# nnethercott/hannoy

Measured on AMD Instinct MI355X. Metric: vectors indexed/sec (build) + recall@10, 1M x 768 Cosine M=16 efC=100, higher is better.
Workload: dtype f32

## Files before the change

hannoy_amd/csrc/hny_host.cpp:

```cpp
#include "../../include/hannoy_amd.h"
#include "hny_internal.h"
#include "hny_rust_sort.h"

#include <malloc.h>
#include <algorithm>
#include <array>
#include <atomic>
#include <mutex>
#include <chrono>
#include <cmath>
#include <cstdarg>
#include <cstdio>
#include <cstdlib>
#include <cstring>
#include <functional>
#include <iterator>
#include <memory>
#include <numeric>
#include <string>
#include <thread>
#include <type_traits>
#include <utility>
#include <vector>

// ... 289 lines not shown
  std::vector<int8_t> ins_level;
  std::vector<uint16_t> old_mask;
  std::vector<uint8_t> deleted;
  std::vector<u64> old_recs;
  bool incremental = false;
  bool load_only = false;
  bool gaps_done = false;
  bool from_update = false;
  uint64_t n_done0 = 0;
  uint32_t up_layers = 1;
  std::vector<uint32_t> entry_points;
  std::vector<uint64_t> rec_first;
  std::vector<uint32_t> rec_item_t;
  std::vector<uint8_t> rec_layer_t;
  std::vector<int32_t> upper_idx;
  uint32_t max_level = 0, n_upper = 0;
  LaunchShape shape{64, 1};
  double frac = 0.0;
  uint32_t bmax = 0;
  int device = 0;
  hipStream_t stream = nullptr;
  std::vector<hipEvent_t> sync_evs;
  size_t sync_used = 0;
  size_t pos = 0;
  uint64_t n_done = 0, n_batches = 0;
  hny_batch cur{};
  bool in_batch = false, finalized = false;
  GraphDev g{};
  DevBuf<unsigned char> d_rows, d_level;
  DevBuf<float> d_norms, d_l0_dist, d_up_dist;
  DevBuf<int> d_upper_idx;
  DevBuf<u32> d_l0_ids, d_l0_cnt, d_up_ids, d_up_cnt, d_order, d_eps, d_bits, d_vlog, d_cand_n,
      d_seg_start, d_nseg, d_deferred, d_deferred_b, d_fin_cnt0, d_fin_cntu, d_d0_ids, d_du_ids;
  DevBuf<unsigned char> d_has_vec, d_deleted;
  DevBuf<u64> d_old_recs, d_lkey_a, d_lkey_b, d_perm_a, d_perm_b;
  DevBuf<u32> d_gap_bitmap, d_gap_bm;
  DevBuf<u64> d_gap_keys, d_gap_sorted;
  int gap_grid = 0;
  DevBuf<u32> d_eps0;
  DevBuf<u32> d_pool_retry, d_pool_retry2, d_pool_ctr;
  DevBuf<u64> d_heap_c, d_heap_r;
  uint32_t heap_grid = 0, heap_c_cap = 0, heap_r_cap = 0, pool_ctr_used = 0;
  uint32_t heap_grid1 = 0, heap_c_cap1 = 0;
  u64 *heap_c_ptr = nullptr;
  struct ExportBufs : ExportSlots {
    std::thread th;
    void join() {
      if (th.joinable()) th.join();
    }
    void drop() {
      join();
      drop_all();
    }
    ~ExportBufs() { drop(); }
  } xbuf;
  bool will_export = true;
  std::vector<uint32_t> item_slot;
  uint64_t n_items = 0;
  std::unique_ptr<IngestPipe> qpipe;
  uint64_t nrec_bound = 0, nbr_bound = 0;
  bool locality = true;
  u32 *h_l0 = nullptr, *h_up = nullptr, *h_cnt0 = nullptr, *h_cntu = nullptr;
  DevBuf<u64> d_stats, d_stats_scratch, d_sel, d_cand, d_res_global;
  DevBuf<u64> d_ops;
  struct { u64 *p = nullptr; size_t n = 0; } d_keys_a, d_keys_b, d_vals_a, d_vals_b;
  DevBuf<unsigned char> d_sort_tmp;
// ... 122 lines not shown
  for (uint32_t v : set)
    if (c <= v) {
      s.lpr = (int)l;
      s.nch = (int)v;
      return HNY_OK;
    }
  return fail(HNY_ERR_UNSUPPORTED, "dim %u needs more than 16 chunks per lane (max f32 dim 4096)", dim);
}

int mclass_of(int metric) {
  switch (metric) {
    case HNY_COSINE: return MC_DOT;
    case HNY_EUCLIDEAN: return MC_L2;
    case HNY_MANHATTAN: return MC_L1;
    default: return MC_BIN;
  }
}

uint32_t cap_of(const hny_builder *b, uint32_t layer_or_level) {
  return layer_or_level == 0 ? b->o.M0 : b->o.M;
}

int env_int(const char *name, int dflt) {
  const char *v = getenv(name);
  return v && *v ? atoi(v) : dflt;
}

Knobs knobs_from_env() {
  Knobs k{};
  k.no_fast = env_int("HNY_NO_FAST", 0) != 0;
  k.no_rb = env_int("HNY_NO_RB", 0) != 0;
  k.rb_one = env_int("HNY_RB_ONE", 1) != 0;
  k.prune_n8 = env_int("HNY_PRUNE_N8", 1) != 0;
  k.walk_slots = env_int("HNY_WALK_SLOTS", HNY_KNOB_UNSET);
  k.xcd_tile = env_int("HNY_XCD_TILE", HNY_KNOB_UNSET);
  k.prune_xcd_tile = env_int("HNY_PRUNE_XCD_TILE", HNY_KNOB_UNSET);
  k.walk_resident = env_int("HNY_WALK_RESIDENT", HNY_KNOB_UNSET);
  k.visited_log = env_int("HNY_VISITED_LOG", HNY_KNOB_UNSET);
  k.vis_slots = env_int("HNY_VIS_SLOTS", HNY_KNOB_UNSET);
  k.stage_bytes = env_int("HNY_STAGE_BYTES", HNY_KNOB_UNSET);
  k.no_locality = env_int("HNY_NO_LOCALITY", 0) != 0;
  k.heap_small_cap = env_int("HNY_HEAP_SMALL_CAP", HNY_KNOB_UNSET);
  k.vis_buckets = env_int("HNY_VIS_BUCKETS", HNY_KNOB_UNSET);
  return k;
}

int upload_rows(const void *vectors, size_t stride, size_t vbytes, uint64_t n, uint32_t row_stride,
                unsigned char *dst, hipStream_t st, const uint32_t *slots = nullptr, uint64_t n_slots = 0) {
  if (!slots) n_slots = n;
  if (!slots && stride == row_stride && vbytes == row_stride) {
    HIP_TRY(hipMemcpyAsync(dst, vectors, (size_t)n * row_stride, hipMemcpyHostToDevice, st));
    HIP_TRY(hipStreamSynchronize(st));
    return HNY_OK;
  }
  const size_t chunk_rows = std::max<size_t>(1, (64u << 20) / row_stride);
  std::vector<unsigned char> stage(chunk_rows * row_stride);
  uint64_t r = 0;
  for (uint64_t s0 = 0; s0 < n_slots; s0 += chunk_rows) {
    size_t cnt = (size_t)std::min<uint64_t>(chunk_rows, n_slots - s0);
    std::fill(stage.begin(), stage.begin() + cnt * row_stride, 0);
    for (; r < n && (slots ? slots[r] : r) < s0 + cnt; r++)
      memcpy(&stage[((slots ? slots[r] : r) - s0) * row_stride], (const unsigned char *)vectors + r * stride, vbytes);
    HIP_TRY(hipMemcpyAsync(dst + s0 * row_stride, stage.data(), cnt * row_stride,
                           hipMemcpyHostToDevice, st));
    HIP_TRY(hipStreamSynchronize(st));
  }
// ... 112 lines not shown
    a.out_hdrs = j.out_hdrs ? p.d_hdrs[k] : nullptr;
    HIP_TRY(hnyk_ingest(a, st));
    HIP_TRY(hipEventRecord(p.consumed[k], st));
    p.used[k] = true;
    if (j.out_codes)
      HIP_TRY(hipMemcpyAsync((unsigned char *)j.out_codes + r0 * vb, p.d_codes[k], (size_t)cnt * vb, hipMemcpyDeviceToHost, st));
    if (j.out_hdrs)
      HIP_TRY(hipMemcpyAsync((unsigned char *)j.out_hdrs + r0 * hb, p.d_hdrs[k], (size_t)cnt * hb, hipMemcpyDeviceToHost, st));
  }
  return HNY_OK;
}

int check_f32_rows(uint32_t dim, uint64_t n, const void *vectors, size_t stride) {
  if (dim == 0) return fail(HNY_ERR_INVALID_DIM, "dim must be > 0");
  if (n && !vectors) return fail(HNY_ERR_INVALID_ARG, "null f32 vectors");
  if (n && stride < (size_t)dim * 4)
    return fail(HNY_ERR_INVALID_DIM, "stride %zu < %zu bytes of f32 for dim %u", stride, (size_t)dim * 4, dim);
  if (n && stride % 4) return fail(HNY_ERR_INVALID_ARG, "f32 stride %zu is not a multiple of 4", stride);
  return HNY_OK;
}

int reset_graph(hny_builder *b) {
  hipStream_t st = b->stream;
  HIP_TRY(hnyk_fill_u32(b->d_l0_ids.p, HNY_SENT, b->d_l0_ids.n, st));
  HIP_TRY(hipMemsetAsync(b->d_l0_cnt.p, 0, b->d_l0_cnt.n * 4, st));
  HIP_TRY(hipMemsetAsync(b->d_l0_dist.p, 0, b->d_l0_dist.n * 4, st));
  if (b->d_up_ids.n) {
    HIP_TRY(hnyk_fill_u32(b->d_up_ids.p, HNY_SENT, b->d_up_ids.n, st));
    HIP_TRY(hipMemsetAsync(b->d_up_cnt.p, 0, b->d_up_cnt.n * 4, st));
    HIP_TRY(hipMemsetAsync(b->d_up_dist.p, 0, b->d_up_dist.n * 4, st));
  }
  HIP_TRY(hipMemsetAsync(b->d_stats.p, 0, ST_COUNT * 8, st));
  HIP_TRY(hipMemsetAsync(b->d_bits.p, 0, b->d_bits.n * 4, st));
  b->pos = 0;
  b->n_done = b->n_done0;
  b->n_batches = 0;
  b->in_batch = false;
  b->finalized = false;
  b->gaps_done = false;
  b->ev_used = 0;
  b->n_walk_dispatch = 0;
  b->sync_used = 0;
  b->t_build0 = now_s();
  return HNY_OK;
}

int use_device(int device) {
  int ndev = 0;
  if (hipGetDeviceCount(&ndev) != hipSuccess || ndev == 0)
    return fail(HNY_ERR_NO_DEVICE, "no HIP device (this library has no CPU path)");
  if (device >= 0) HIP_TRY(hipSetDevice(device));
  return HNY_OK;
}

size_t group_end(const hny_builder *b, size_t pos) {
  size_t e = pos;
  while (e < b->order.size() && b->order_level[e] == b->order_level[pos]) e++;
  return e;
}

inline uint32_t rec_mask_of(const hny_builder *b, uint32_t s) {
  if (b->deleted[s]) return 0u;
  uint32_t m = b->old_mask[s];
  if (b->ins_level[s] >= 0) m |= (2u << b->ins_level[s]) - 1u;
  return m;
}
// ... 751 lines not shown
    const uint64_t area = b->heap_c_ptr == b->d_ops.p ? b->d_ops.n : b->d_heap_c.n;
    const uint64_t small_cap = (uint64_t)std::max(16, knob_or(b->knobs.heap_small_cap, 1 << 18));
    if ((uint64_t)b->heap_c_cap > small_cap) {
      b->heap_c_cap1 = (uint32_t)small_cap;
      b->heap_grid1 = (uint32_t)std::max<uint64_t>(1, std::min<uint64_t>(std::min<uint64_t>(slots, 512), area / small_cap));
      HIP_TRY(b->d_pool_retry2.alloc(cand_rows));
    }
    HIP_TRY(b->d_heap_r.alloc((size_t)std::max(b->heap_grid, b->heap_grid1) * b->heap_r_cap));
    HIP_TRY(b->d_pool_retry.alloc(cand_rows));
    HIP_TRY(b->d_pool_ctr.alloc(4 * 64));
  }
  HIP_TRY(b->d_deferred.alloc(b->max_ops));
  HIP_TRY(b->d_deferred_b.alloc(b->max_ops));
  {
    u32 tbits = 1;
    while ((1ull << tbits) < (u64)b->n + 1ull) tbits++;
    const u32 ranges[3][2] = {{0, 64}, {HNY_SEQ_BITS, 64}, {HNY_SEQ_BITS, (u32)HNY_SEQ_BITS + tbits}};
    b->sort_tmp_bytes = 0;
    for (size_t sz = b->max_ops; sz >= 1; sz = sz > 1 ? sz / 2 : 0) {
      for (auto &r : ranges) {
        size_t need = 0;
        HIP_TRY(hnyk_sort_pairs(nullptr, need, b->d_keys_a.p, b->d_keys_b.p, b->d_vals_a.p, b->d_vals_b.p,
                                (u32)sz, r[0], r[1], st));
        b->sort_tmp_bytes = std::max(b->sort_tmp_bytes, need);
      }
      size_t need = 0;
      HIP_TRY(hnyk_sort_pairs48(nullptr, need, b->d_keys_a.p, b->d_keys_b.p, b->d_vals_a.p, b->d_vals_b.p,
                                (u32)sz, st));
      b->sort_tmp_bytes = std::max(b->sort_tmp_bytes, need);
      need = 0;
      HIP_TRY(hnyk_sort_u32(nullptr, need, b->d_deferred.p, b->d_deferred_b.p, (u32)sz, st));
      b->sort_tmp_bytes = std::max(b->sort_tmp_bytes, need);
      if (sz == 1) break;
    }
  }
  HIP_TRY(b->d_sort_tmp.alloc(b->sort_tmp_bytes + 16));
  if (b->incremental && n) {
    HIP_TRY(b->d_d0_ids.alloc((size_t)n * o.M0));
    HIP_TRY(b->d_du_ids.alloc(std::max<size_t>(nup * o.M, 1)));
    HIP_TRY(b->d_has_vec.alloc(n));
    HIP_TRY(b->d_deleted.alloc(n));
    HIP_TRY(b->d_old_recs.alloc(std::max<size_t>(b->old_recs.size(), 1)));
  }

  GraphDev &g = b->g;
  const size_t vb = vec_bytes(o.metric, o.dim);
  g.n = n;
  g.metric = o.metric;
  g.mclass = mclass_of(o.metric);
  g.row_stride = row_stride;
  g.bin_bits = (u32)(vb * 8);
  g.bin_inv = (g.bin_bits && (g.bin_bits & (g.bin_bits - 1)) == 0) ? 1.0f / (float)g.bin_bits : 0.0f;
  g.M = o.M;
  g.M0 = o.M0;
  g.max_level = b->max_level;
  g.up_layers = b->up_layers;
  g.n_upper = b->n_upper;
  g.alpha = o.alpha;
  g.incremental = b->incremental ? 1 : 0;
  g.dim = o.dim;
  g.x86_order = o.x86_order ? 1 : 0;
  g.rows = b->d_rows.p;
  g.norms = b->d_norms.p;
  g.level = b->d_level.p;
  g.upper_idx = b->d_upper_idx.p;
  g.l0_ids = b->d_l0_ids.p;
// ... 375 lines not shown
      prof_end(b);
      PruneArgs p = prune_args(l, lo, hi);
      p.perm = b->d_perm_b.p;
      prof_begin(b, EV_PRUNE);
      HIP_TRY(launch_prune(p, b->stream));
      prof_end(b);
    }
    return HNY_OK;
  }
  for (int32_t l = (int32_t)L; l >= 0; l--) {
    WalkArgs w = walk_args(l, lo, hi, queues + l);
    prof_begin(b, EV_WALK);
    b->n_walk_dispatch++;
    HIP_TRY(launch_walk(w, b->stream));
    prof_end(b);
    prof_begin(b, EV_PRUNE);
    HIP_TRY(launch_prune(prune_args(l, lo, hi), b->stream));
    prof_end(b);
  }
  return HNY_OK;
}

static int apply_front(hny_builder *b, const void *sel_dev, ApplyArgs &a) {
  const uint32_t L = b->cur.level, cs = cap_of(b, L);
  const u64 *sel = sel_dev ? (const u64 *)sel_dev : b->d_sel.p;
  const u32 n_ops = b->cur.count * (L + 1) * cs * 2;
  EmitArgs e{};
  e.q_slots = b->d_order.p + b->cur.first;
  e.count = b->cur.count;
  e.sel = sel;
  e.sel_stride = b->cur.sel_stride_u64;
  e.cap_sel = cs;
  e.batch_level = L;
  e.keys = b->d_keys_a.p;
  e.vals = b->d_vals_a.p;
  prof_begin(b, EV_SORT);
  HIP_TRY(hnyk_emit(b->g, e, b->stream));
  size_t tmp = b->sort_tmp_bytes;
  HIP_TRY(hnyk_sort_pairs(b->d_sort_tmp.p, tmp, b->d_keys_a.p, b->d_keys_b.p, b->d_vals_a.p,
                          b->d_vals_b.p, n_ops, 0, 64, b->stream));
  HIP_TRY(hipMemsetAsync(b->d_nseg.p, 0, 8, b->stream));
  HIP_TRY(hnyk_segments(b->d_keys_b.p, n_ops, b->d_seg_start.p, b->d_nseg.p, b->stream));
  prof_end(b);
  a = ApplyArgs{};
  a.keys = b->d_keys_b.p;
  a.vals = b->d_vals_b.p;
  a.n_ops = n_ops;
  a.seg_start = b->d_seg_start.p;
  a.n_seg = b->d_nseg.p;
  a.deferred = b->apply_form.kind == APPLY_WAVE ? nullptr : b->d_deferred.p;
  a.n_deferred = b->d_nseg.p + 1;
  prof_begin(b, EV_APPLY);
  if (a.deferred) {
    HIP_TRY(hnyk_apply_append(b->g, a, b->stream));
  } else {
    const int grid = (int)std::min<u32>(std::max<u32>(n_ops / 2, 1), b->apply_form.grid_cap);
    HIP_TRY(hnyk_apply(b->g, a, b->shape, b->apply_form, grid, b->stream));
  }
  prof_end(b);
  b->cur_n_ops = n_ops;
  return HNY_OK;
}

static void apply_back(hny_builder *b) {
  b->pos += b->cur.count;
  b->n_done += b->cur.count;
  b->n_batches++;
  b->in_batch = false;
  b->apply_open = false;
}

int hny_builder_apply(hny_builder *b, const void *sel_dev) {
  if (!b || !b->in_batch || b->apply_open) return fail(HNY_ERR_INVALID_ARG, "no current batch");
  HIP_TRY(hipSetDevice(b->device));
  ApplyArgs a;
// ... 2592 lines not shown
```

hannoy_amd/csrc/hny_internal.h:

```cpp
#pragma once
#include <hip/hip_runtime.h>
#include <stddef.h>
#include <stdint.h>

typedef unsigned long long u64;
typedef unsigned int u32;

#define HNY_SENT 0xFFFFFFFFu
#define HNY_MAX_CAP 64
#define HNY_BIG_CAP 1024
#define HNY_MAX_EPS 8192
#define HNY_POOL_CAP 128
#define HNY_MAX_EF 65535
#define HNY_OP_INVALID 0xFFFFFFFFFFFFFFFFull
#define HNY_SEQ_BITS 29
#define HNY_MAX_LEVEL 14

enum { MC_DOT = 0, MC_L2 = 1, MC_L1 = 2, MC_BIN = 3 };

enum {
  ST_EVALS_WALK = 0,
  ST_EVALS_PRUNE = 1,
  ST_EVALS_APPLY = 2,
  ST_LINKS = 3,
// ... 144 lines not shown
  u32 count;
  const u64 *sel;
  u32 sel_stride, cap_sel, batch_level;
  u64 *keys;
  u64 *vals;
};

struct ApplyArgs {
  const u64 *keys;
  const u64 *vals;
  u32 n_ops;
  const u32 *seg_start;
  const u32 *n_seg;
  u32 *deferred;
  u32 *n_deferred;
  u32 shard_rank, shard_world;
  u64 *exch;
  u32 exch_stride;
};

struct LaunchShape {
  int lpr;
  int nch;
};

#define HNY_KNOB_UNSET (-2147483647 - 1)
struct Knobs {
  int no_fast;
  int no_rb;
  int rb_one;
  int prune_n8;
  int walk_slots, xcd_tile, prune_xcd_tile, walk_resident, visited_log, vis_slots, stage_bytes, no_locality,
      heap_small_cap, vis_buckets;
};
static inline int knob_or(int v, int dflt) { return v == HNY_KNOB_UNSET ? dflt : v; }

#ifndef HNY_RB_MAX_NCH
#define HNY_RB_MAX_NCH 3
#endif
#ifndef HNY_WALK_WPE
#define HNY_WALK_WPE 4
#endif
#ifndef HNY_WALK_WPE_SMALL
#define HNY_WALK_WPE_SMALL 6
#endif
constexpr int hnyk_walk_waves_per_simd(int lpr, int nch, int sp, bool rm, int rc) {
  return nch == 1 && sp >= 4 && !rm && (rc == 1 || rc == 2) && lpr <= 32 ? HNY_WALK_WPE_SMALL : HNY_WALK_WPE;
}

static inline bool hnyk_fast_path(const GraphDev &g, const Knobs &k) {
  return !k.no_fast && !g.x86_order && !g.incremental && g.metric >= 0 && g.metric < 7 && g.M0 <= 64u;
}
struct WalkForm {
  int sp;
  bool big_eps;
  bool reader;
  int rc;
  int waves_per_simd;
};
static inline WalkForm hnyk_walk_form(const GraphDev &g, const WalkArgs &a, LaunchShape s, const Knobs &k) {
  WalkForm f{0, a.eps_cap > 64, false, 0, 0};
  if (hnyk_fast_path(g, k) && a.eps_cap <= 64 && !a.res_global) {
    f.sp = g.metric + 1;
    f.reader = a.reader_mode != 0;
    if (s.nch <= HNY_RB_MAX_NCH && a.rcap <= 128 && !k.no_rb)
      f.rc = s.nch == 1 && s.lpr <= 32 && !f.reader && a.rb_one && k.rb_one ? 1 : 2;
// ... 81 lines not shown
  const u32 *filter_of;
  const u32 *masks;
  u32 mask_stride;
  const u32 *k_of;
  u32 *tile_mask;
};
static inline u32 hnyk_exact_qt(u32 row_stride) {
  u32 qt = 32;
  while (qt > 4 && (size_t)qt * row_stride > 65536u) qt /= 2;
  return qt;
}
hipError_t hnyk_exact_scores(const GraphDev &g, const ExactArgs &a, LaunchShape s, hipStream_t st);
hipError_t hnyk_exact_topk(const GraphDev &g, const ExactArgs &a, hipStream_t st);
hipError_t hnyk_exact_tile_masks(const ExactArgs &a, hipStream_t st);
struct RangeArgs {
  const float *scores;
  u32 score_stride;
  u32 nq;
  u32 slab_base, slab_n;
  const u32 *mask;
  const float *radius;
  u64 *count;
  u64 *keys;
  const u32 *seg;
  u32 *cursor;
};
hipError_t hnyk_range_count(const RangeArgs &a, hipStream_t st);
hipError_t hnyk_range_emit(const RangeArgs &a, hipStream_t st);
hipError_t hnyk_range_sort(void *temp, size_t &temp_bytes, u64 *keys, u64 *other, u32 n, u32 n_seg, const u32 *seg,
                           u64 **sorted, hipStream_t st);
hipError_t hnyk_range_finish(const u64 *keys, u32 n, const u32 *item_ids, u32 *ids, u32 *dist_bits, hipStream_t st);
hipError_t hnyk_emit(const GraphDev &g, const EmitArgs &a, hipStream_t st);
hipError_t hnyk_segments(const u64 *keys, u32 n_ops, u32 *seg_start, u32 *n_seg, hipStream_t st);
hipError_t hnyk_apply(const GraphDev &g, const ApplyArgs &a, LaunchShape s, const ApplyForm &f, int grid, hipStream_t st);
hipError_t hnyk_apply_append(const GraphDev &g, const ApplyArgs &a, hipStream_t st);
hipError_t hnyk_apply_deferred(const GraphDev &g, const ApplyArgs &a, LaunchShape s, const ApplyForm &f, StageRows sl,
                               u32 work, hipStream_t st);
hipError_t hnyk_apply_merge(const GraphDev &g, const u64 *exch, u32 n_def, u32 world, u32 rank, u32 per,
                            u32 stride, hipStream_t st);
hipError_t hnyk_sort_u32(void *temp, size_t &temp_bytes, u32 *in, u32 *out, u32 n, hipStream_t st);
hipError_t hnyk_sort_pairs(void *temp, size_t &temp_bytes, u64 *keys_in, u64 *keys_out, u64 *vals_in,
                           u64 *vals_out, u32 n, u32 begin_bit, u32 end_bit, hipStream_t st);
hipError_t hnyk_sort_pairs48(void *temp, size_t &temp_bytes, u64 *keys_in, u64 *keys_out, u64 *vals_in,
                             u64 *vals_out, u32 n, hipStream_t st);
hipError_t hnyk_iota_u64(u64 *p, u32 base, u32 n, hipStream_t st);
hipError_t hnyk_take_topk(const u64 *cand, const u32 *cand_n, u32 rcap, u32 k, u32 n, u64 *out,
                          hipStream_t st);
hipError_t hnyk_lane_selftest(u32 *out64, hipStream_t st);
hipError_t hnyk_pair_distances(const GraphDev &g, const u32 *a, const u32 *b, u32 n, float *out,
                               LaunchShape s, hipStream_t st);
hipError_t hnyk_fill_u32(u32 *p, u32 v, size_t n, hipStream_t st);
hipError_t hnyk_fill_gaps_wg(const GraphDev &g, const u64 *recs, u32 n_recs, const unsigned char *deleted,
                             u32 *bitmaps, u32 words, u32 *bm, u32 maxb, u64 *keys, u64 *sorted, int SL, int grid,
                             LaunchShape s, hipStream_t st);
hipError_t hnyk_fill_gaps(const GraphDev &g, const u64 *recs, u32 n_recs, const unsigned char *deleted,
                          LaunchShape s, hipStream_t st);
hipError_t hnyk_finalize_lists(u32 *ids, u32 *cnt_out, u32 n_lists, u32 cap, hipStream_t st);
size_t hnyk_walk_lds_bytes(u32 rcap, u32 eps_cap);
#define HNY_DECL_SP(N)                                                                                         \
  hipError_t hnyk_walk_sp##N(const GraphDev &g, const WalkArgs &a, LaunchShape s, const WalkForm &f, int grid, \
                             hipStream_t st);                                                                  \
  hipError_t hnyk_prune_sp##N(const GraphDev &g, const PruneArgs &a, LaunchShape s, const PruneForm &f, int SL, \
                              int grid, hipStream_t st);                                                       \
  hipError_t hnyk_apply_sp##N(const GraphDev &g, const ApplyArgs &a, LaunchShape s, const ApplyForm &f, int SL, \
                              int grid, hipStream_t st);
HNY_DECL_SP(1) HNY_DECL_SP(2) HNY_DECL_SP(3) HNY_DECL_SP(4) HNY_DECL_SP(5) HNY_DECL_SP(6) HNY_DECL_SP(7)
// ... 59 lines not shown
```

hannoy_amd/csrc/hny_kernels.hip:

```cpp
#include "hny_internal.h"

#include <algorithm>
#include <cstdlib>
#include <cstring>
#ifndef HNY_PART
#define HNY_PART 0
#endif
#if HNY_PART == 0
#include <rocprim/device/device_radix_sort.hpp>
#endif

#ifdef HNY_WSYNC_BARRIER
#define WSYNC() __syncthreads()
#else
#define WSYNC()                                               \
  do {                                                        \
    __builtin_amdgcn_fence(__ATOMIC_RELEASE, "workgroup");    \
    __builtin_amdgcn_wave_barrier();                          \
    __builtin_amdgcn_fence(__ATOMIC_ACQUIRE, "workgroup");    \
  } while (0)
#endif

#ifndef HNY_RB_MERGE
#define HNY_RB_MERGE 1
#endif
#ifndef HNY_RB_MERGE_MIN
#define HNY_RB_MERGE_MIN 2
#endif

#define HNY_LANE ((int)(threadIdx.x & 63u))

namespace {

__device__ __forceinline__ u32 fbits(float f) { return __float_as_uint(f); }
__device__ __forceinline__ u64 ballot(bool p) { return __builtin_amdgcn_ballot_w64(p); }

template <int SP>
__device__ __forceinline__ void specialize(GraphDev &g) {
  if constexpr (SP != 0) {
    g.metric = SP - 1;
    g.mclass = SP - 1 < 3 ? SP - 1 : (int)MC_BIN;
    g.x86_order = 0;
    g.incremental = 0;
  }
}
__device__ __forceinline__ u32 uni(u32 x) { return (u32)__builtin_amdgcn_readfirstlane((int)x); }
__device__ __forceinline__ u64 uni64(u64 x) { return ((u64)uni((u32)(x >> 32)) << 32) | (u64)uni((u32)x); }
__device__ __forceinline__ int uni(int x) { return __builtin_amdgcn_readfirstlane(x); }
__device__ __forceinline__ u64 uni(u64 x) {
  return ((u64)uni((u32)(x >> 32)) << 32) | (u64)uni((u32)(x & 0xFFFFFFFFull));
}

template <int LPR, int NCH>
__device__ __forceinline__ void load_row(const unsigned char *p, int t, u32 n16, float4 (&r)[NCH]) {
// ... 3283 lines not shown
    for (int j = 0; j < 4; j++) k[j + 1] = i0 + (u32)j < n_ops ? keys[i0 + j] : HNY_OP_INVALID;
    u32 flags = 0u;
#pragma unroll
    for (int j = 0; j < 4; j++) {
      const bool start = k[j + 1] != HNY_OP_INVALID &&
                         ((i0 + (u32)j) == 0u || (k[j] >> HNY_SEQ_BITS) != (k[j + 1] >> HNY_SEQ_BITS));
      flags |= (start ? 1u : 0u) << j;
    }
    const u32 c = (u32)__popc(flags);
    u32 incl = c;
#pragma unroll
    for (int off = 1; off < 64; off <<= 1) {
      const u32 t = (u32)__shfl_up((int)incl, off, 64);
      if (ln >= off) incl += t;
    }
    if (ln == 63) wsum[w] = incl;
    __syncthreads();
    u32 wbase = 0u, total = 0u;
#pragma unroll
    for (int j = 0; j < 4; j++) {
      if (j < w) wbase += wsum[j];
      total += wsum[j];
    }
    if (tid == 0) base_s = total ? atomicAdd(n_seg, total) : 0u;
    __syncthreads();
    u32 pos = base_s + wbase + incl - c;
#pragma unroll
    for (int j = 0; j < 4; j++)
      if ((flags >> j) & 1u) seg_start[pos++] = i0 + (u32)j;
    __syncthreads();
  }
}

__global__ __launch_bounds__(256) void k_apply_append(GraphDev g, ApplyArgs a) {
  const u32 n_seg = *a.n_seg;
  for (u32 sg = blockIdx.x * blockDim.x + threadIdx.x; sg < n_seg; sg += gridDim.x * blockDim.x) {
    const u32 i0 = a.seg_start[sg];
    const u64 k0 = a.keys[i0] >> HNY_SEQ_BITS;
    const u32 target = (u32)(k0 & 0x7FFFFFFFull);
    const NodeList l = node_list(g, (u32)(k0 >> 31), target);
    const u32 cw = *l.cnt;
    if (cw >> 31) continue;
    u32 cnt = cw & 0xFFFFu;
    u32 nops = 0;
    for (u32 i = i0; i < a.n_ops; i++) {
      const u64 key = a.keys[i];
      if (key == HNY_OP_INVALID || (key >> HNY_SEQ_BITS) != k0) break;
      nops++;
      if (cnt + nops > l.cap) break;
    }
    if (cnt + nops > l.cap) {
      a.deferred[atomicAdd(a.n_deferred, 1u)] = i0;
      continue;
    }
    for (u32 i = i0; i < i0 + nops; i++) {
      const u64 val = a.vals[i];
      if ((u32)(val & 0xFFFFFFFFull) == target) continue;
      l.ids[cnt] = (u32)(val & 0xFFFFFFFFull);
      l.dist[cnt] = __uint_as_float((u32)(val >> 32));
      cnt++;
    }
    *l.cnt = cnt;
  }
}

template <int LPR, int NCH, int SP>
// ... 776 lines not shown
                               u32 work, hipStream_t st) {
  const int SL = f.kind == APPLY_APPEND_N8 ? sl.n8 : sl.wg, grid = (int)std::min<u32>(work, f.grid_cap);
  HNY_SP_SWITCH(f.sp, hnyk_apply_sp, g, a, s, f, SL, grid, st)
  return dispatch_shape<Hot<0>::Apply>(s, g, a, f, SL, grid, st);
}
hipError_t hnyk_pair_distances(const GraphDev &g, const u32 *a, const u32 *b, u32 n, float *out,
                               LaunchShape s, hipStream_t st) {
  return dispatch_shape<PairLauncher>(s, g, a, b, n, out, st);
}
hipError_t hnyk_fill_gaps(const GraphDev &g, const u64 *recs, u32 n_recs, const unsigned char *deleted,
                          LaunchShape s, hipStream_t st) {
  if (!n_recs) return hipSuccess;
  return dispatch_shape<GapsLauncher>(s, g, recs, n_recs, deleted, st);
}
hipError_t hnyk_fill_gaps_wg(const GraphDev &g, const u64 *recs, u32 n_recs, const unsigned char *deleted,
                             u32 *bitmaps, u32 words, u32 *bm, u32 maxb, u64 *keys, u64 *sorted, int SL, int grid,
                             LaunchShape s, hipStream_t st) {
  if (!n_recs) return hipSuccess;
  return dispatch_shape<GapsWgLauncher>(s, g, recs, n_recs, deleted, bitmaps, words, bm, maxb, keys, sorted, SL,
                                        grid, st);
}
hipError_t hnyk_emit(const GraphDev &g, const EmitArgs &a, hipStream_t st) {
  u64 total = (u64)a.count * (a.batch_level + 1) * a.cap_sel;
  if (!total) return hipSuccess;
  hipLaunchKernelGGL(k_emit, dim3((unsigned)std::min<u64>((total + 255) / 256, 2048)), dim3(256), 0, st, g, a);
  return hipGetLastError();
}
hipError_t hnyk_segments(const u64 *keys, u32 n_ops, u32 *seg_start, u32 *n_seg, hipStream_t st) {
  if (!n_ops) return hipSuccess;
  hipLaunchKernelGGL(k_segments, dim3(std::min<u32>((n_ops + 1023) / 1024, 2048u)), dim3(256), 0, st, keys,
                     n_ops, seg_start, n_seg);
  return hipGetLastError();
}
hipError_t hnyk_apply_append(const GraphDev &g, const ApplyArgs &a, hipStream_t st) {
  if (!a.n_ops) return hipSuccess;
  hipLaunchKernelGGL(k_apply_append, dim3(std::min<u32>((a.n_ops / 2 + 255) / 256, 4096u)), dim3(256), 0, st, g, a);
  return hipGetLastError();
}
hipError_t hnyk_finalize_lists(u32 *ids, u32 *cnt_out, u32 n_lists, u32 cap, hipStream_t st) {
  if (!n_lists) return hipSuccess;
  unsigned grid = n_lists < 65536u * 4u ? n_lists : 65536u * 4u;
  hipLaunchKernelGGL(k_finalize_lists, dim3(grid), dim3(64), 0, st, ids, cnt_out, n_lists, cap);
  return hipGetLastError();
}
hipError_t hnyk_ingest(const IngestArgs &a, hipStream_t st) {
  if (!a.cnt) return hipSuccess;
  const bool bits = a.codec == ING_BINARY || a.codec == ING_BQ;
  const bool src16 = a.src_stride % 4u == 0 && ((uintptr_t)a.src & 15u) == 0;
  const bool v4 = src16 && (bits || !a.out_codes || (a.dim % 4u == 0 && ((uintptr_t)a.out_codes & 15u) == 0));
  const u32 rows_per_block = bits ? 16u : 32u;
  const unsigned grid = (unsigned)std::min<u64>(((u64)a.cnt + rows_per_block - 1) / rows_per_block, 8192);
  if (a.src_of) {
    if (!src16 || a.src_stride * 4u < (a.dim + 3u) / 4u * 16u) return hipErrorInvalidValue;
    if (bits) hipLaunchKernelGGL((k_ingest_bits<true, true>), dim3(grid), dim3(256), 0, st, a);
    else if (v4) hipLaunchKernelGGL((k_ingest_f32<true, true>), dim3(grid), dim3(256), 0, st, a);
    else hipLaunchKernelGGL((k_ingest_f32<false, true>), dim3(grid), dim3(256), 0, st, a);
    return hipGetLastError();
  }
  if (bits) {
    if (v4) hipLaunchKernelGGL(k_ingest_bits<true>, dim3(grid), dim3(256), 0, st, a);
    else hipLaunchKernelGGL(k_ingest_bits<false>, dim3(grid), dim3(256), 0, st, a);
  } else {
    if (v4) hipLaunchKernelGGL(k_ingest_f32<true>, dim3(grid), dim3(256), 0, st, a);
    else hipLaunchKernelGGL(k_ingest_f32<false>, dim3(grid), dim3(256), 0, st, a);
  }
  return hipGetLastError();
// ... 120 lines not shown
```

Before: 2.579 million.

## Replace radix sort of link ops with per-list counting sort and local ordering

Link operations emitted per batch are now bucketed into per-list slots with a count pass, an exclusive scan of offsets, and a fill pass, instead of a full 64-bit radix sort followed by segment detection. Each list's small segment is then ordered in place with a wave-level rank sort, and lists longer than 64 entries go through a separate chunked pass. The goal is to avoid the multi-pass radix sort cost on large batches. In exchange it adds atomics, several extra launches, and a scan over all lists (n + upper lists) every batch, so small batches keep the old sort path through a size threshold.

```diff
diff --git a/hannoy_amd/csrc/hny_host.cpp b/hannoy_amd/csrc/hny_host.cpp
--- a/hannoy_amd/csrc/hny_host.cpp
+++ b/hannoy_amd/csrc/hny_host.cpp
@@ -345,6 +345,7 @@
   DevBuf<int> d_upper_idx;
   DevBuf<u32> d_l0_ids, d_l0_cnt, d_up_ids, d_up_cnt, d_order, d_eps, d_bits, d_vlog, d_cand_n,
       d_seg_start, d_nseg, d_deferred, d_deferred_b, d_fin_cnt0, d_fin_cntu, d_d0_ids, d_du_ids;
+  DevBuf<u32> d_link_cnt, d_link_off;
   DevBuf<unsigned char> d_has_vec, d_deleted;
   DevBuf<u64> d_old_recs, d_lkey_a, d_lkey_b, d_perm_a, d_perm_b;
   DevBuf<u32> d_gap_bitmap, d_gap_bm;
@@ -533,6 +534,7 @@
   k.no_rb = env_int("HNY_NO_RB", 0) != 0;
   k.rb_one = env_int("HNY_RB_ONE", 1) != 0;
   k.prune_n8 = env_int("HNY_PRUNE_N8", 1) != 0;
+  k.link_sort = env_int("HNY_LINK_SORT", HNY_KNOB_UNSET);
   k.walk_slots = env_int("HNY_WALK_SLOTS", HNY_KNOB_UNSET);
   k.xcd_tile = env_int("HNY_XCD_TILE", HNY_KNOB_UNSET);
   k.prune_xcd_tile = env_int("HNY_PRUNE_XCD_TILE", HNY_KNOB_UNSET);
@@ -711,6 +713,7 @@
   }
   HIP_TRY(hipMemsetAsync(b->d_stats.p, 0, ST_COUNT * 8, st));
   HIP_TRY(hipMemsetAsync(b->d_bits.p, 0, b->d_bits.n * 4, st));
+  if (b->d_link_cnt.n) HIP_TRY(hipMemsetAsync(b->d_link_cnt.p, 0, b->d_link_cnt.n * 4, st));
   b->pos = 0;
   b->n_done = b->n_done0;
   b->n_batches = 0;
@@ -1528,6 +1531,15 @@
       HIP_TRY(hnyk_sort_u32(nullptr, need, b->d_deferred.p, b->d_deferred_b.p, (u32)sz, st));
       b->sort_tmp_bytes = std::max(b->sort_tmp_bytes, need);
       if (sz == 1) break;
+    }
+    if ((u64)n + nup + 1 > 0xFFFFFFFFull) b->knobs.link_sort = 1;
+    if (b->knobs.link_sort != 1) {
+      HIP_TRY(b->d_link_cnt.alloc((size_t)n + nup + 1));
+      HIP_TRY(b->d_link_off.alloc((size_t)n + nup + 1));
+      HIP_TRY(hipMemsetAsync(b->d_link_cnt.p, 0, b->d_link_cnt.n * 4, st));
+      size_t need = 0;
+      HIP_TRY(hnyk_link_offsets(nullptr, need, b->d_link_cnt.p, b->d_link_off.p, (u32)(n + nup), st));
+      b->sort_tmp_bytes = std::max(b->sort_tmp_bytes, need);
     }
   }
   HIP_TRY(b->d_sort_tmp.alloc(b->sort_tmp_bytes + 16));
@@ -1969,15 +1981,32 @@
   e.sel_stride = b->cur.sel_stride_u64;
   e.cap_sel = cs;
   e.batch_level = L;
-  e.keys = b->d_keys_a.p;
-  e.vals = b->d_vals_a.p;
   prof_begin(b, EV_SORT);
-  HIP_TRY(hnyk_emit(b->g, e, b->stream));
+  HIP_TRY(hipMemsetAsync(b->d_nseg.p, 0, 12, b->stream));
   size_t tmp = b->sort_tmp_bytes;
-  HIP_TRY(hnyk_sort_pairs(b->d_sort_tmp.p, tmp, b->d_keys_a.p, b->d_keys_b.p, b->d_vals_a.p,
-                          b->d_vals_b.p, n_ops, 0, 64, b->stream));
-  HIP_TRY(hipMemsetAsync(b->d_nseg.p, 0, 8, b->stream));
-  HIP_TRY(hnyk_segments(b->d_keys_b.p, n_ops, b->d_seg_start.p, b->d_nseg.p, b->stream));
+  const u32 n_lists = b->d_link_cnt.n ? (u32)b->d_link_cnt.n - 1 : 0u;
+  const bool counting = b->knobs.link_sort == 0 ||
+                        (b->knobs.link_sort == HNY_KNOB_UNSET && n_ops >= std::max<u32>(HNY_LINK_COUNT_MIN_SLOTS, n_lists / 16));
+  if (counting) {
+    e.keys = b->d_keys_b.p;
+    e.vals = b->d_vals_b.p;
+    u32 *rank = (u32 *)b->d_keys_a.p, *fwd = (u32 *)b->d_vals_a.p;
+    HIP_TRY(hnyk_link_count(b->g, e, b->d_link_cnt.p, fwd, rank, b->stream));
+    HIP_TRY(hnyk_link_offsets(b->d_sort_tmp.p, tmp, b->d_link_cnt.p, b->d_link_off.p, n_lists, b->stream));
+    HIP_TRY(hnyk_link_fill(b->g, e, b->d_link_off.p, fwd, rank, b->stream));
+#ifdef HNY_LINK_MEMSET_RESET
+    HIP_TRY(hipMemsetAsync(b->d_link_cnt.p, 0, b->d_link_cnt.n * 4, b->stream));
+#endif
+    HIP_TRY(hnyk_link_order(b->d_link_off.p, b->d_link_cnt.p, n_lists, b->d_keys_b.p, b->d_vals_b.p, b->d_keys_a.p, b->d_vals_a.p,
+                            b->d_deferred_b.p, b->d_nseg.p + 2, b->d_seg_start.p, b->d_nseg.p, n_ops, b->stream));
+  } else {
+    e.keys = b->d_keys_a.p;
+    e.vals = b->d_vals_a.p;
+    HIP_TRY(hnyk_emit(b->g, e, b->stream));
+    HIP_TRY(hnyk_sort_pairs(b->d_sort_tmp.p, tmp, b->d_keys_a.p, b->d_keys_b.p, b->d_vals_a.p,
+                            b->d_vals_b.p, n_ops, 0, 64, b->stream));
+    HIP_TRY(hnyk_segments(b->d_keys_b.p, n_ops, b->d_seg_start.p, b->d_nseg.p, b->stream));
+  }
   prof_end(b);
   a = ApplyArgs{};
   a.keys = b->d_keys_b.p;
diff --git a/hannoy_amd/csrc/hny_internal.h b/hannoy_amd/csrc/hny_internal.h
--- a/hannoy_amd/csrc/hny_internal.h
+++ b/hannoy_amd/csrc/hny_internal.h
@@ -200,6 +200,7 @@
   int prune_n8;
   int walk_slots, xcd_tile, prune_xcd_tile, walk_resident, visited_log, vis_slots, stage_bytes, no_locality,
       heap_small_cap, vis_buckets;
+  int link_sort;
 };
 static inline int knob_or(int v, int dflt) { return v == HNY_KNOB_UNSET ? dflt : v; }
 
@@ -347,6 +348,14 @@
 hipError_t hnyk_range_finish(const u64 *keys, u32 n, const u32 *item_ids, u32 *ids, u32 *dist_bits, hipStream_t st);
 hipError_t hnyk_emit(const GraphDev &g, const EmitArgs &a, hipStream_t st);
 hipError_t hnyk_segments(const u64 *keys, u32 n_ops, u32 *seg_start, u32 *n_seg, hipStream_t st);
+#define HNY_LINK_COUNT_MIN_SLOTS 16384u
+#define HNY_LINK_LONG_GRID 512u
+#define HNY_LINK_ORDER_GRID 1024u
+hipError_t hnyk_link_count(const GraphDev &g, const EmitArgs &a, u32 *cnt, u32 *fwd, u32 *rank, hipStream_t st);
+hipError_t hnyk_link_offsets(void *temp, size_t &temp_bytes, u32 *cnt, u32 *off, u32 n_lists, hipStream_t st);
+hipError_t hnyk_link_fill(const GraphDev &g, const EmitArgs &a, const u32 *off, u32 *fwd, u32 *rank, hipStream_t st);
+hipError_t hnyk_link_order(const u32 *off, u32 *cnt, u32 n_lists, u64 *keys, u64 *vals, u64 *tmp_keys, u64 *tmp_vals,
+                           u32 *items, u32 *n_items, u32 *seg_start, u32 *n_seg, u32 n_slots, hipStream_t st);
 hipError_t hnyk_apply(const GraphDev &g, const ApplyArgs &a, LaunchShape s, const ApplyForm &f, int grid, hipStream_t st);
 hipError_t hnyk_apply_append(const GraphDev &g, const ApplyArgs &a, hipStream_t st);
 hipError_t hnyk_apply_deferred(const GraphDev &g, const ApplyArgs &a, LaunchShape s, const ApplyForm &f, StageRows sl,
diff --git a/hannoy_amd/csrc/hny_kernels.hip b/hannoy_amd/csrc/hny_kernels.hip
--- a/hannoy_amd/csrc/hny_kernels.hip
+++ b/hannoy_amd/csrc/hny_kernels.hip
@@ -8,6 +8,7 @@
 #endif
 #if HNY_PART == 0
 #include <rocprim/device/device_radix_sort.hpp>
+#include <rocprim/device/device_scan.hpp>
 #endif
 
 #ifdef HNY_WSYNC_BARRIER
@@ -20,6 +21,13 @@
     __builtin_amdgcn_fence(__ATOMIC_ACQUIRE, "workgroup");    \
   } while (0)
 #endif
+
+#define WAVE_SYNC()                                           \
+  do {                                                        \
+    __builtin_amdgcn_fence(__ATOMIC_RELEASE, "workgroup");    \
+    __builtin_amdgcn_wave_barrier();                          \
+    __builtin_amdgcn_fence(__ATOMIC_ACQUIRE, "workgroup");    \
+  } while (0)
 
 #ifndef HNY_RB_MERGE
 #define HNY_RB_MERGE 1
@@ -3369,6 +3377,156 @@
   }
 }
 
+__device__ __forceinline__ u32 list_index(const GraphDev &g, u32 layer, u32 node) {
+  return layer == 0 ? node : g.n + (u32)g.upper_idx[node] * g.up_layers + (layer - 1);
+}
+
+template <bool FILL>
+__global__ __launch_bounds__(256) void k_link_ops(GraphDev g, EmitArgs a, u32 *cnt, const u32 *off, u32 *fwd, u32 *rank) {
+  const u32 n_layers = a.batch_level + 1;
+  const u64 total = (u64)a.count * n_layers * a.cap_sel;
+  const u64 stride = (u64)gridDim.x * blockDim.x;
+  u64 links = 0;
+  for (u64 idx = (u64)blockIdx.x * blockDim.x + threadIdx.x; idx < total; idx += stride) {
+    const u32 k = (u32)(idx % a.cap_sel);
+    const u32 li = (u32)((idx / a.cap_sel) % n_layers);
+    const u32 m = (u32)(idx / ((u64)a.cap_sel * n_layers));
+    const u64 *s = a.sel + (size_t)m * a.sel_stride + (size_t)li * (a.cap_sel + 1);
+    const u32 s0 = min((u32)s[0], a.cap_sel);
+    if (k >= s0) continue;
+    const u64 e = s[1 + k];
+    const u32 nb = (u32)(e & 0xFFFFFFFFull), q = a.q_slots[m];
+    const u32 layer = a.batch_level - li;
+    const u32 lq = list_index(g, layer, q), lt = list_index(g, layer, nb);
+    if constexpr (!FILL) {
+      if (k == 0) fwd[(size_t)m * n_layers + li] = atomicAdd(&cnt[lq], s0);
+      rank[idx] = atomicAdd(&cnt[lt], 1u);
+      links += 2;
+    } else {
+      const u64 o = idx * 2, db = e >> 32;
+      const u32 pq = off[lq] + fwd[(size_t)m * n_layers + li] + k;
+      a.keys[pq] = ((u64)layer << (31 + HNY_SEQ_BITS)) | ((u64)q << HNY_SEQ_BITS) | o;
+      a.vals[pq] = (db << 32) | nb;
+      const u32 pn = off[lt] + rank[idx];
+      a.keys[pn] = ((u64)layer << (31 + HNY_SEQ_BITS)) | ((u64)nb << HNY_SEQ_BITS) | (o + 1);
+      a.vals[pn] = (db << 32) | q;
+    }
+  }
+  if constexpr (!FILL) {
+#pragma unroll
+    for (int sh = 32; sh >= 1; sh >>= 1) links += (u64)__shfl_xor((long long)links, sh, 64);
+    if ((threadIdx.x & 63) == 0 && links) atomicAdd(&g.stats[ST_LINKS], links);
+  }
+}
+
+__device__ __forceinline__ u32 wave_rank_key(const u64 *keys, u32 s, u32 n, u64 mine, u64 *chunk) {
+  const u32 ln = (u32)HNY_LANE;
+  u32 rank = 0;
+  for (u32 c0 = 0; c0 < n; c0 += 64u) {
+    chunk[ln] = c0 + ln < n ? keys[s + c0 + ln] : HNY_OP_INVALID;
+    WAVE_SYNC();
+#pragma unroll 8
+    for (int j = 0; j < 64; j++) rank += chunk[j] < mine ? 1u : 0u;
+    WAVE_SYNC();
+  }
+  return rank;
+}
+
+template <bool COPY>
+__global__ __launch_bounds__(256) void k_link_long(const u32 *items, const u32 *n_items, u64 *keys, u64 *vals, u64 *tk,
+                                                   u64 *tv) {
+  __shared__ u64 chunk[4][64];
+  const u32 ln = threadIdx.x & 63u, w = threadIdx.x >> 6;
+  const u32 ni = *n_items;
+  for (u32 it = blockIdx.x * 4u + w; it < ni; it += gridDim.x * 4u) {
+    const u32 s = items[3 * it], n = items[3 * it + 1], e = items[3 * it + 2] + ln;
+    if constexpr (COPY) {
+      if (e < n) {
+        keys[s + e] = tk[s + e];
+        vals[s + e] = tv[s + e];
+      }
+    } else {
+      const u64 mine = e < n ? keys[s + e] : HNY_OP_INVALID;
+      const u32 rank = wave_rank_key(keys, s, n, mine, chunk[w]);
+      if (e < n) {
+        tk[s + rank] = mine;
+        tv[s + rank] = vals[s + e];
+      }
+    }
+  }
+}
+
+__global__ __launch_bounds__(256) void k_link_order(const u32 *off, u32 *cnt, u32 n_lists, u64 *keys, u64 *vals,
+                                                    u32 *items, u32 *n_items, u32 *seg_start, u32 *n_seg, u32 n_slots) {
+  __shared__ u32 wsum[4];
+  __shared__ u32 base_s, n_long;
+  __shared__ u32 long_s[256], long_n[256];
+  __shared__ u64 chunk[4][64];
+  const int tid = threadIdx.x, ln = tid & 63, w = tid >> 6;
+  if (blockIdx.x == 0 && tid == 0) {
+    const u32 total = off[n_lists];
+    if (total < n_slots) keys[total] = HNY_OP_INVALID;
+  }
+  for (u32 b0 = blockIdx.x * 256u; b0 < n_lists; b0 += gridDim.x * 256u) {
+    if (tid == 0) n_long = 0u;
+    __syncthreads();
+    const u32 i = b0 + (u32)tid;
+    u32 s = 0u, n = 0u;
+    if (i < n_lists) {
+      s = off[i];
+      n = off[i + 1] - s;
+    }
+    const u64 has = ballot(n > 0u);
+    if (ln == 0) wsum[w] = (u32)__popcll(has);
+#ifndef HNY_LINK_MEMSET_RESET
+    if (n > 0u) cnt[i] = 0u;
+#endif
+    if (n == 2u) {
+      const u64 k0 = keys[s], k1 = keys[s + 1];
+      if (k0 > k1) {
+        const u64 v0 = vals[s], v1 = vals[s + 1];
+        keys[s] = k1;
+        keys[s + 1] = k0;
+        vals[s] = v1;
+        vals[s + 1] = v0;
+      }
+    } else if (n > 64u) {
+      const u32 nc = (n + 63u) / 64u;
+      const u32 c0 = atomicAdd(n_items, nc);
+      for (u32 c = 0; c < nc; c++) {
+        items[3 * (c0 + c)] = s;
+        items[3 * (c0 + c) + 1] = n;
+        items[3 * (c0 + c) + 2] = c * 64u;
+      }
+    } else if (n > 2u) {
+      const u32 j = atomicAdd(&n_long, 1u);
+      long_s[j] = s;
+      long_n[j] = n;
+    }
+    __syncthreads();
+    u32 wbase = 0u, total = 0u;
+#pragma unroll
+    for (int j = 0; j < 4; j++) {
+      if (j < w) wbase += wsum[j];
+      total += wsum[j];
+    }
+    if (tid == 0) base_s = total ? atomicAdd(n_seg, total) : 0u;
+    __syncthreads();
+    if (n > 0u) seg_start[base_s + wbase + (u32)__popcll(has & ((1ull << ln) - 1ull))] = s;
+    for (u32 j = (u32)w; j < n_long; j += 4u) {
+      const u32 ss = long_s[j], nn = long_n[j];
+      const u64 mine = (u32)ln < nn ? keys[ss + ln] : HNY_OP_INVALID;
+      const u64 val = (u32)ln < nn ? vals[ss + ln] : 0ull;
+      const u32 rank = wave_rank_key(keys, ss, nn, mine, chunk[w]);
+      if ((u32)ln < nn) {
+        keys[ss + rank] = mine;
+        vals[ss + rank] = val;
+      }
+    }
+    __syncthreads();
+  }
+}
+
 __global__ __launch_bounds__(256) void k_apply_append(GraphDev g, ApplyArgs a) {
   const u32 n_seg = *a.n_seg;
   for (u32 sg = blockIdx.x * blockDim.x + threadIdx.x; sg < n_seg; sg += gridDim.x * blockDim.x) {
@@ -4211,6 +4369,32 @@
                      n_ops, seg_start, n_seg);
   return hipGetLastError();
 }
+hipError_t hnyk_link_count(const GraphDev &g, const EmitArgs &a, u32 *cnt, u32 *fwd, u32 *rank, hipStream_t st) {
+  const u64 total = (u64)a.count * (a.batch_level + 1) * a.cap_sel;
+  if (!total) return hipSuccess;
+  hipLaunchKernelGGL(k_link_ops<false>, dim3((unsigned)std::min<u64>((total + 255) / 256, 2048)), dim3(256), 0, st, g,
+                     a, cnt, (const u32 *)nullptr, fwd, rank);
+  return hipGetLastError();
+}
+hipError_t hnyk_link_offsets(void *temp, size_t &temp_bytes, u32 *cnt, u32 *off, u32 n_lists, hipStream_t st) {
+  return rocprim::exclusive_scan(temp, temp_bytes, cnt, off, 0u, (size_t)n_lists + 1, rocprim::plus<u32>(), st);
+}
+hipError_t hnyk_link_fill(const GraphDev &g, const EmitArgs &a, const u32 *off, u32 *fwd, u32 *rank, hipStream_t st) {
+  const u64 total = (u64)a.count * (a.batch_level + 1) * a.cap_sel;
+  if (!total) return hipSuccess;
+  hipLaunchKernelGGL(k_link_ops<true>, dim3((unsigned)std::min<u64>((total + 255) / 256, 2048)), dim3(256), 0, st, g,
+                     a, (u32 *)nullptr, off, fwd, rank);
+  return hipGetLastError();
+}
+hipError_t hnyk_link_order(const u32 *off, u32 *cnt, u32 n_lists, u64 *keys, u64 *vals, u64 *tmp_keys, u64 *tmp_vals,
+                           u32 *items, u32 *n_items, u32 *seg_start, u32 *n_seg, u32 n_slots, hipStream_t st) {
+  if (!n_lists) return hipSuccess;
+  hipLaunchKernelGGL(k_link_order, dim3(std::min<u32>((n_lists + 255) / 256, HNY_LINK_ORDER_GRID)), dim3(256), 0, st,
+                     off, cnt, n_lists, keys, vals, items, n_items, seg_start, n_seg, n_slots);
+  hipLaunchKernelGGL(k_link_long<false>, dim3(HNY_LINK_LONG_GRID), dim3(256), 0, st, items, n_items, keys, vals, tmp_keys, tmp_vals);
+  hipLaunchKernelGGL(k_link_long<true>, dim3(HNY_LINK_LONG_GRID), dim3(256), 0, st, items, n_items, keys, vals, tmp_keys, tmp_vals);
+  return hipGetLastError();
+}
 hipError_t hnyk_apply_append(const GraphDev &g, const ApplyArgs &a, hipStream_t st) {
   if (!a.n_ops) return hipSuccess;
   hipLaunchKernelGGL(k_apply_append, dim3(std::min<u32>((a.n_ops / 2 + 255) / 256, 4096u)), dim3(256), 0, st, g, a);
```

Measured after the change: 2.603 million (median of 6 runs). Within noise of the previous version (+0.9%).
